# andrewendlinger/xmris

Measured on AMD Instinct MI355X. Metric: spectra/sec (zero_fill->apodize->FFT->autophase), n_time=4096; HBM-roofline %, higher is better.
Workload: dtype f32

## Files before the change

xmris_amd/csrc/xm_coarse.h:

```cpp
#pragma once
#include "xm_kernels.h"

typedef _Float16 xm_h8 __attribute__((ext_vector_type(8)));
typedef _Float16 xm_h2 __attribute__((ext_vector_type(2)));
typedef float xm_f16v __attribute__((ext_vector_type(16)));

struct CoarseArgs {
  const void* in;
  const float* window;
  const Cx<float>* w1024;
  float* est;
  unsigned long long* gkey;
  long long in_stride;
  long long n_batch;
  float scale2;
};

constexpr int kCoarseWaves = 4;

XM_DEV Cx<float> coarse_w1024(const Cx<float>* __restrict__ t, unsigned k) {
  k &= 1023u;
  const Cx<float> w = t[k & 511u];
  return (k & 512u) ? mk<float>(-w.re, -w.im) : w;
}

XM_DEV xm_h8 coarse_pack(const float* v) {
  union {
    xm_h8 v8;
    xm_h2 v2[4];
  } u;
#pragma unroll
  for (int j = 0; j < 4; ++j) {
    const xm_f2 p = {v[2 * j], v[2 * j + 1]};
    u.v2[j] = __builtin_convertvector(p, xm_h2);
  }
  return u.v8;
}

template <bool IN64>
__global__ __launch_bounds__(64 * kCoarseWaves, 2) void k_coarse_mfma(CoarseArgs A) {
  const unsigned lane = threadIdx.x & 63u, r = lane & 31u, h = lane >> 5;
  const long long wave = (long long)blockIdx.x * kCoarseWaves + (threadIdx.x >> 6);
  const long long n_waves = (long long)gridDim.x * kCoarseWaves;

  xm_h8 b1r, b1i, b1n, a2r[2], a2i[2], a2n[2];
  {
    float cr[8], ci[8], cn[8];
#pragma unroll
    for (int j = 0; j < 8; ++j) {
      const Cx<float> w = coarse_w1024(A.w1024, 32u * ((8u * h + (unsigned)j) * r));
      cr[j] = w.re;
      ci[j] = w.im;
      cn[j] = -w.im;
    }
    b1r = coarse_pack(cr);
    b1i = coarse_pack(ci);
    b1n = coarse_pack(cn);
#pragma unroll
    for (int s = 0; s < 2; ++s) {
#pragma unroll
      for (int j = 0; j < 8; ++j) {
        const unsigned n2 = 16u * s + 8u * ((unsigned)j >> 2) + 4u * h + ((unsigned)j & 3u);
        const Cx<float> w = coarse_w1024(A.w1024, 32u * (n2 * r));
        cr[j] = w.re;
        ci[j] = w.im;
        cn[j] = -w.im;
      }
      a2r[s] = coarse_pack(cr);
      a2i[s] = coarse_pack(ci);
      a2n[s] = coarse_pack(cn);
    }
  }
  float twr[16], twi[16];
#pragma unroll
  for (int q = 0; q < 16; ++q) {
    const unsigned n2 = ((unsigned)q & 3u) + 8u * ((unsigned)q >> 2) + 4u * h;
    const Cx<float> w = coarse_w1024(A.w1024, n2 * r);
    twr[q] = w.re;
    twi[q] = w.im;
  }
  float wnd[8];
#pragma unroll
  for (int j = 0; j < 8; ++j) wnd[j] = A.window[32u * (8u * h + (unsigned)j) + r];

  auto fetch = [&](long long s, Cx<float>* x) {
    if constexpr (IN64) {
      const xm_d2* __restrict__ row = reinterpret_cast<const xm_d2*>(A.in) + s * A.in_stride;
#pragma unroll
      for (int j = 0; j < 8; ++j) {
        const xm_d2 v = __builtin_nontemporal_load(row + 32u * (8u * h + (unsigned)j) + r);
        x[j] = mk<float>((float)v.x, (float)v.y);
      }
      return;
    }
    const xm_f2* __restrict__ row = reinterpret_cast<const xm_f2*>(A.in) + s * A.in_stride;
#pragma unroll
    for (int j = 0; j < 8; ++j) {
      const xm_f2 v = __builtin_nontemporal_load(row + 32u * (8u * h + (unsigned)j) + r);
      x[j] = mk<float>(v.x, v.y);
    }
  };

  unsigned best_key = 0u, best_row = 0u;
  bool have = false;
  constexpr int DEPTH = 1;
  Cx<float> nx[DEPTH][8];
  long long s = wave;
#pragma unroll
  for (int d = 0; d < DEPTH; ++d)
    if (s + d * n_waves < A.n_batch) fetch(s + d * n_waves, nx[d]);
  auto one_row = [&](Cx<float>* cur, long long s) {
    float re[8], im[8];
    float m = 0.f;
#pragma unroll
    for (int j = 0; j < 8; ++j) {
      re[j] = cur[j].re * wnd[j];
      im[j] = cur[j].im * wnd[j];
      m = fmaxf(m, fmaxf(fabsf(re[j]), fabsf(im[j])));
    }
    if (s + DEPTH * n_waves < A.n_batch) fetch(s + DEPTH * n_waves, cur);
    unsigned e = (wave_reduce_u32<true>(__float_as_uint(m)) >> 23) & 0xffu;
    e = e > 253u ? 253u : (e < 1u ? 1u : e);
    const float up = __uint_as_float((254u - e) << 23);
    const float down = __uint_as_float(e << 23);
#pragma unroll
    for (int j = 0; j < 8; ++j) {
      re[j] *= up;
      im[j] *= up;
    }
    const xm_h8 ar = coarse_pack(re), ai = coarse_pack(im);
    xm_f16v d1r = {0.f}, d1i = {0.f};
    d1r = __builtin_amdgcn_mfma_f32_32x32x16_f16(ar, b1r, d1r, 0, 0, 0);
    d1r = __builtin_amdgcn_mfma_f32_32x32x16_f16(ai, b1n, d1r, 0, 0, 0);
    d1i = __builtin_amdgcn_mfma_f32_32x32x16_f16(ar, b1i, d1i, 0, 0, 0);
    d1i = __builtin_amdgcn_mfma_f32_32x32x16_f16(ai, b1r, d1i, 0, 0, 0);
    float zr[16], zi[16];
#pragma unroll
    for (int q = 0; q < 16; ++q) {
      zr[q] = d1r[q] * twr[q] - d1i[q] * twi[q];
      zi[q] = d1r[q] * twi[q] + d1i[q] * twr[q];
    }
    xm_f16v d2r = {0.f}, d2i = {0.f};
#pragma unroll
    for (int k = 0; k < 2; ++k) {
      const xm_h8 br = coarse_pack(zr + 8 * k), bi = coarse_pack(zi + 8 * k);
      d2r = __builtin_amdgcn_mfma_f32_32x32x16_f16(a2r[k], br, d2r, 0, 0, 0);
      d2r = __builtin_amdgcn_mfma_f32_32x32x16_f16(a2n[k], bi, d2r, 0, 0, 0);
      d2i = __builtin_amdgcn_mfma_f32_32x32x16_f16(a2r[k], bi, d2i, 0, 0, 0);
      d2i = __builtin_amdgcn_mfma_f32_32x32x16_f16(a2i[k], br, d2i, 0, 0, 0);
    }
    float bv = -1.f;
#pragma unroll
    for (int q = 0; q < 16; ++q) bv = fmaxf(bv, d2r[q] * d2r[q] + d2i[q] * d2i[q]);
    bv = amax_nan_if_unset(bv);
    bv = bv * (down * down) * A.scale2;
    const unsigned key = wave_reduce_u32<true>(bv != bv ? 0x7fc00000u : __float_as_uint(bv));
    const unsigned row = (unsigned)s;
    const bool take = !have || key > best_key;
    best_key = take ? key : best_key;
    best_row = take ? row : best_row;
    have = true;
    if (lane == 0u) A.est[s] = __uint_as_float(key);
  };
  for (; s < A.n_batch; s += DEPTH * n_waves) {
#pragma unroll
    for (int d = 0; d < DEPTH; ++d)
      if (s + d * n_waves < A.n_batch) one_row(nx[d], s + d * n_waves);
  }
  if (A.gkey && have && lane == 0u)
    atomicMax(A.gkey + (blockIdx.x % XM_KEY_SLOTS) * XM_KEY_STRIDE,
              ((unsigned long long)best_key << 32) | (unsigned long long)(0xffffffffu - best_row));
}
```

xmris_amd/device.py:

```python
from __future__ import annotations

import numpy as np

from . import _lib


def _torch():
    import torch

    return torch


def _dtype_code(x) -> int:
    torch = _torch()
    if x.dtype == torch.complex64:
        return _lib.XM_C64
    if x.dtype == torch.complex128:
        return _lib.XM_C128
    raise TypeError(f"xmris_amd kernels need complex64/complex128 data, got {x.dtype}")


def _real_dtype(x):
    torch = _torch()
    return torch.float32 if x.dtype == torch.complex64 else torch.float64


def _require_device(x):
    torch = _torch()
    if not isinstance(x, torch.Tensor):
        raise TypeError("expected a torch.Tensor resident on the GPU")
    if not x.is_cuda:
        raise RuntimeError(
            "xmris_amd has no CPU path: the tensor must live on a HIP device (use xmris_amd.to_device)"
        )


def _stream(x):
    torch = _torch()
    return torch.cuda.current_stream(x.device).cuda_stream


def to_device(a, device="cuda", dtype=None):
    torch = _torch()
    if isinstance(a, torch.Tensor):
        t = a
    else:
        a = np.asarray(a)
        if not np.iscomplexobj(a):
            a = a.astype(np.complex128 if a.dtype != np.float32 else np.complex64)
        t = torch.from_numpy(np.ascontiguousarray(a))
    if dtype is not None:
        t = t.to(dtype)
    if not t.is_complex():
        t = t.to(torch.complex128 if t.dtype == torch.float64 else torch.complex64)
    return t.to(device)


_HOST_STAGE = {}
_HOST_STAGE_BUFS = 4
_HOST_STAGE_LOCK = __import__("threading").Lock()


def to_host(x, chunk_bytes: int = 32 << 20):
    torch = _torch()
    x = x.detach()
    nbytes = x.numel() * x.element_size()
    if not x.is_cuda or nbytes < 4 * chunk_bytes:
        return x.cpu().numpy()
    with _HOST_STAGE_LOCK:
        return _to_host_staged(x.contiguous(), chunk_bytes)


def _to_host_staged(x, chunk_bytes: int):
    torch = _torch()
    from concurrent.futures import ThreadPoolExecutor

    nbytes = x.numel() * x.element_size()
    dev_idx = x.device.index or 0
    if dev_idx not in _HOST_STAGE:
        _HOST_STAGE[dev_idx] = ([torch.empty(chunk_bytes, dtype=torch.uint8, pin_memory=True)
                                 for _ in range(_HOST_STAGE_BUFS)],
                                torch.cuda.Stream(device=x.device), ThreadPoolExecutor(max_workers=_HOST_STAGE_BUFS))
    stage, side, pool = _HOST_STAGE[dev_idx]
    np_dtype = {torch.complex64: np.complex64, torch.complex128: np.complex128, torch.float32: np.float32,
                torch.float64: np.float64}.get(x.dtype)
    if np_dtype is None or chunk_bytes != stage[0].numel():
        return x.cpu().numpy()
    out = np.empty(tuple(x.shape), dtype=np_dtype)
    dst = out.reshape(-1).view(np.uint8)
    src = (torch.view_as_real(x) if x.is_complex() else x).reshape(-1).view(torch.uint8)
    stage_np = [b.numpy() for b in stage]
    side.wait_stream(torch.cuda.current_stream(x.device))
    pending = [None] * len(stage)

    def drain(ev, lo, n, k):
        ev.synchronize()
        np.copyto(dst[lo:lo + n], stage_np[k][:n])

    for i, lo in enumerate(range(0, nbytes, chunk_bytes)):
        k, n = i % len(stage), min(chunk_bytes, nbytes - lo)
        if pending[k] is not None:
            pending[k].result()
        with torch.cuda.stream(side):
            stage[k][:n].copy_(src[lo:lo + n], non_blocking=True)
            ev = torch.cuda.Event()
            ev.record(side)
        pending[k] = pool.submit(drain, ev, lo, n, k)
    for f in pending:
        if f is not None:
            f.result()
    x.record_stream(side)
    return out


def _rows(x, axis):
    nd = x.dim()
    axis = axis % nd
    xm = x.movedim(axis, -1) if axis != nd - 1 else x
    lead = tuple(xm.shape[:-1])
    n = xm.shape[-1]
    x2 = xm.reshape(-1, n)
    if not x2.is_contiguous():
        x2 = x2.contiguous()

    def restore(y2):
        y = y2.reshape(lead + (y2.shape[-1],))
        if axis != nd - 1:
            y = y.movedim(-1, axis).contiguous()
        return y

    return x2, restore


def _table(values, like, complex_table: bool):
    torch = _torch()
    if isinstance(values, torch.Tensor):
        t = values
    else:
        t = torch.from_numpy(np.ascontiguousarray(np.asarray(values)))
    want = like.dtype if complex_table else _real_dtype(like)
    return t.to(device=like.device, dtype=want).contiguous()


def zero_fill(x, axis: int, target_points: int, pad_left: int = 0):
    _require_device(x)
    torch = _torch()
    x2, restore = _rows(x, axis)
    nb, n_in = x2.shape
    out = torch.empty((nb, target_points), dtype=x.dtype, device=x.device)
    _lib.call("xm_zero_fill", x2.data_ptr(), out.data_ptr(), nb, n_in, target_points, pad_left,
              _dtype_code(x), _stream(x))
    return restore(out)


def apodize(x, axis: int, window):
    _require_device(x)
    torch = _torch()
    x2, restore = _rows(x, axis)
    nb, n = x2.shape
    w = _table(window, x, complex_table=False)
    if w.numel() != n:
        raise ValueError(f"window has {w.numel()} points, axis has {n}")
    out = torch.empty_like(x2)
    _lib.call("xm_apodize", x2.data_ptr(), out.data_ptr(), w.data_ptr(), nb, n, _dtype_code(x), _stream(x))
    return restore(out)


def zf_apod_supported(n_out: int, out_complex128: bool) -> bool:
    return int(n_out) * (8 if out_complex128 else 4) <= 96 * 1024


def zf_apod(x2, n_out: int, pad_left: int, window, promote: bool = False):
    _require_device(x2)
    torch = _torch()
    if x2.dim() != 2 or not x2.is_contiguous():
        raise ValueError("zf_apod expects a contiguous [n_batch, n_in] tensor")
    nb, n_in = x2.shape
    out_dt = torch.complex128 if (promote or x2.dtype == torch.complex128) else torch.complex64
    rd = torch.float64 if out_dt == torch.complex128 else torch.float32
    if isinstance(window, torch.Tensor):
        w = window.to(device=x2.device, dtype=rd).contiguous()
    else:
        w = torch.from_numpy(np.ascontiguousarray(np.asarray(window, dtype=np.float64))).to(device=x2.device, dtype=rd)
    if w.numel() != n_out:
        raise ValueError(f"window has {w.numel()} points, the zero-filled axis has {n_out}")
    out = torch.empty((nb, n_out), dtype=out_dt, device=x2.device)
    _lib.call("xm_zf_apod", x2.data_ptr(), n_in, out.data_ptr(), w.data_ptr(), nb, n_in, int(n_out), int(pad_left),
              _dtype_code(x2), _lib.XM_C128 if out_dt == torch.complex128 else _lib.XM_C64, _stream(x2))
    return out


def phase_apply(x, axis: int, table):
    _require_device(x)
    torch = _torch()
    x2, restore = _rows(x, axis)
    nb, n = x2.shape
    ph = _table(table, x, complex_table=True)
    if ph.numel() != n:
        raise ValueError(f"phase table has {ph.numel()} points, axis has {n}")
    out = torch.empty_like(x2)
    _lib.call("xm_phase_apply", x2.data_ptr(), out.data_ptr(), ph.data_ptr(), nb, n, _dtype_code(x),
              _stream(x))
    return restore(out)


def roll(x, axis: int, shift: int):
    _require_device(x)
    torch = _torch()
    x2, restore = _rows(x, axis)
    nb, n = x2.shape
    out = torch.empty_like(x2)
    _lib.call("xm_roll", x2.data_ptr(), out.data_ptr(), nb, n, int(shift) % n, _dtype_code(x), _stream(x))
    return restore(out)


def fft(x, axis: int, inverse: bool = False, ortho: bool = True, shift_in: bool = False,
        shift_out: bool = False):
    _require_device(x)
    torch = _torch()
    x2, restore = _rows(x, axis)
    nb, n = x2.shape
    if n == 1:
        return restore(x2.clone())
    flags = ((_lib.XM_FFT_INVERSE if inverse else 0) | (_lib.XM_FFT_ORTHO if ortho else 0)
             | (_lib.XM_FFT_SHIFT_IN if shift_in else 0) | (_lib.XM_FFT_SHIFT_OUT if shift_out else 0))
    out = torch.empty_like(x2)
    _lib.call("xm_fft1d_batched", x2.data_ptr(), out.data_ptr(), nb, n, flags, _dtype_code(x), _stream(x))
    return restore(out)


def slice_axis(x, axis: int, start: int):
    _require_device(x)
    idx = [slice(None)] * x.dim()
    idx[axis % x.dim()] = slice(int(start), None)
    return x[tuple(idx)].contiguous()


def shift_fractional(x, axis: int, start: int, table):
    _require_device(x)
    torch = _torch()
    x2, restore = _rows(x, axis)
    nb, n = x2.shape
    m = n - int(start)
    ph = _table(table, x, complex_table=True)
    if ph.numel() != m:
        raise ValueError(f"table has {ph.numel()} points, sliced axis has {m}")
    view = x2[:, int(start):]
    spec = torch.empty((nb, m), dtype=x.dtype, device=x.device)
    code, st = _dtype_code(x), _stream(x)
    _lib.call("xm_pipeline_fused", view.data_ptr(), n, spec.data_ptr(), None, ph.data_ptr(), nb, m, m, 0, 0,
              None, None, code, st)
    out = torch.empty_like(spec)
    _lib.call("xm_fft1d_batched", spec.data_ptr(), out.data_ptr(), nb, m, _lib.XM_FFT_INVERSE, code, st)
    return restore(out)


def baseline_als(x, axis: int, lam: float, p: float, n_iter: int):
    torch = _torch()
    if not isinstance(x, torch.Tensor) or not x.is_cuda:
        raise RuntimeError("xmris_amd has no CPU path: the tensor must live on a HIP device")
    is_complex = x.is_complex()
    if x.dtype in (torch.complex64, torch.float32):
        code = _lib.XM_C64
    elif x.dtype in (torch.complex128, torch.float64):
        code = _lib.XM_C128
    else:
        raise TypeError(f"baseline_als needs float32/float64 (complex) data, got {x.dtype}")
    x2, restore = _rows(x, axis)
    nb, n = x2.shape
    need = int(_lib.load().xm_baseline_als_workspace_bytes(nb, n))
    work = torch.empty(max(need // 8, 1), dtype=torch.float64, device=x.device)
    out = torch.empty((nb, n), dtype=torch.float64, device=x.device)
    _lib.call("xm_baseline_als", x2.data_ptr(), int(is_complex), nb, n, float(lam), float(p), int(n_iter),
              out.data_ptr(), work.data_ptr(), need, code, torch.cuda.current_stream(x.device).cuda_stream)
    return restore(out)


def amares_model(params, n: int, dt: float, t0: float):
    torch = _torch()
    _require_device(params)
    p = params.to(torch.float64).contiguous()
    if p.dim() < 2 or p.shape[-1] != 5:
        raise ValueError(f"amares_model needs parameters [..., n_peaks, 5], got {tuple(p.shape)}")
    lead, k = tuple(p.shape[:-2]), p.shape[-2]
    nb = int(np.prod(lead, dtype=np.int64)) if lead else 1
    out = torch.empty(lead + (n,), dtype=torch.complex128, device=p.device)
    _lib.call("xm_amares_model", p.data_ptr(), nb, k, int(n), float(dt), float(t0), out.data_ptr(), _stream(p))
    return out


class AmaresFit:

    __slots__ = ("params", "amp_sd", "rss", "status", "iters", "fit", "n_free")

    def __init__(self, **kw):
        for k, v in kw.items():
            setattr(self, k, v)


def amares_fit(x, axis: int, init, lo, hi, fixed, dt: float, t0: float = 0.0, max_iter: int = 200,
               ftol: float = 1e-10, xtol: float = 1e-10, want_fit: bool = True) -> AmaresFit:
    torch = _torch()
    _require_device(x)
    code = _dtype_code(x)
    init, lo, hi = (np.ascontiguousarray(np.asarray(v, dtype=np.float64).reshape(-1, 5)) for v in (init, lo, hi))
    fixed = np.ascontiguousarray(np.asarray(fixed, dtype=bool).reshape(-1, 5).astype(np.int32))
    k = init.shape[0]
    if not (lo.shape == hi.shape == fixed.shape == init.shape):
        raise ValueError("init, lo, hi and fixed must all be [n_peaks, 5]")
    axis = axis % x.dim()
    x2, restore = _rows(x, axis)
    nb, n = x2.shape
    lead = tuple(s for i, s in enumerate(x.shape) if i != axis)
    dev_ = x.device
    params = torch.empty((nb, k, 5), dtype=torch.float64, device=dev_)
    asd = torch.empty((nb, k), dtype=torch.float64, device=dev_)
    rss = torch.empty(nb, dtype=torch.float64, device=dev_)
    status = torch.empty(nb, dtype=torch.int32, device=dev_)
    iters = torch.empty(nb, dtype=torch.int32, device=dev_)
    fit = torch.empty((nb, n), dtype=torch.complex128, device=dev_) if want_fit else None
    need = int(_lib.load().xm_amares_workspace_bytes(nb, n, k))
    work = torch.zeros(max(need, 8), dtype=torch.uint8, device=dev_)
    ptr = lambda a: a.ctypes.data
    _lib.call("xm_amares_fit", x2.data_ptr(), n, nb, n, float(dt), float(t0), k, ptr(init), ptr(lo), ptr(hi), ptr(fixed),
              int(max_iter), float(ftol), float(xtol), params.data_ptr(), asd.data_ptr(), rss.data_ptr(),
              status.data_ptr(), iters.data_ptr(), fit.data_ptr() if fit is not None else None, work.data_ptr(), need,
              code, _stream(x))
    n_free = int(np.count_nonzero(~(fixed.astype(bool) | (lo == hi))))
    return AmaresFit(params=params.reshape(lead + (k, 5)), amp_sd=asd.reshape(lead + (k,)), rss=rss.reshape(lead),
                     status=status.reshape(lead), iters=iters.reshape(lead),
                     fit=fit.reshape(lead + (n,)) if fit is not None else None, n_free=n_free)


def absmax_argmax(x):
    _require_device(x)
    torch = _torch()
    xc = x if x.is_contiguous() else x.contiguous()
    n = xc.shape[-1] if xc.dim() else 1
    x2 = xc.reshape(-1, n)
    nb = x2.shape[0]
    rd = _real_dtype(x)
    amax = torch.empty(nb, dtype=rd, device=x.device)
    aidx = torch.empty(nb, dtype=torch.int32, device=x.device)
    gmax = torch.empty(1, dtype=rd, device=x.device)
    gflat = torch.empty(1, dtype=torch.int64, device=x.device)
    code, st = _dtype_code(x), _stream(x)
    _lib.call("xm_absmax_rows", x2.data_ptr(), nb, n, amax.data_ptr(), aidx.data_ptr(), code, st)
    _lib.call("xm_argmax_reduce", amax.data_ptr(), aidx.data_ptr(), nb, n, gmax.data_ptr(), gflat.data_ptr(),
              code, st)
    return float(gmax.item()) ** 0.5, int(gflat.item())


class FusedResult:

    __slots__ = ("out", "absmax2", "argidx")

    def __init__(self, out, absmax2, argidx):
        self.out, self.absmax2, self.argidx = out, absmax2, argidx


def ramp_native(x2, n_out: int, pad_left: int = 0, shift_out: bool = True, ortho: bool = True) -> bool:
    _require_device(x2)
    flags = (_lib.XM_FFT_ORTHO if ortho else 0) | (_lib.XM_FFT_SHIFT_OUT if shift_out else 0)
    return bool(_lib.load().xm_pipeline_ramp_native(x2.data_ptr(), x2.shape[1], x2.shape[1], int(n_out), int(pad_left),
                                                    flags, _dtype_code(x2)))


def key_native(x2, n_out: int, pad_left: int = 0, shift_out: bool = True, ortho: bool = True) -> bool:
    _require_device(x2)
    flags = (_lib.XM_FFT_ORTHO if ortho else 0) | (_lib.XM_FFT_SHIFT_OUT if shift_out else 0)
    return x2.shape[0] >= 2 and bool(_lib.load().xm_pipeline_key_native(x2.data_ptr(), x2.shape[1], x2.shape[1], int(n_out),
                                                                       int(pad_left), flags, _dtype_code(x2)))


def pipeline_fused(x2, n_out: int, pad_left: int = 0, window=None, phase_table=None, shift_out: bool = True,
                   ortho: bool = True, want_out: bool = True, want_argmax: bool = False, out=None,
                   absmax2=None, argidx=None, argmax_value_only: bool = False, phase_ramp=None, global_key=None,
                   key_result=None):
    _require_device(x2)
    torch = _torch()
    if x2.dim() != 2 or not x2.is_contiguous():
        raise ValueError("pipeline_fused expects a contiguous [n_batch, n_in] tensor")
    nb, n_in = x2.shape
    rd = _real_dtype(x2)
    if want_out and out is None:
        out = torch.empty((nb, n_out), dtype=x2.dtype, device=x2.device)
    if global_key is not None:
        want_argmax, absmax2 = True, global_key
        argidx = key_result
    if want_argmax:
        if absmax2 is None:
            absmax2 = torch.empty(nb, dtype=rd, device=x2.device)
        if argidx is None and global_key is None:
            argidx = torch.empty(nb, dtype=torch.int32, device=x2.device)
    flags = (_lib.XM_FFT_ORTHO if ortho else 0) | (_lib.XM_FFT_SHIFT_OUT if shift_out else 0)
    if global_key is not None:
        flags |= _lib.XM_AMAX_GLOBAL_KEY | _lib.XM_AMAX_VALUE_ONLY
    if argmax_value_only:
        flags |= _lib.XM_AMAX_VALUE_ONLY
    if phase_ramp is not None:
        if phase_table is not None or not want_out:
            raise ValueError("phase_ramp excludes phase_table and needs an output")
        _lib.call(
            "xm_pipeline_fused_ramp", x2.data_ptr(), n_in, out.data_ptr(),
            window.data_ptr() if window is not None else None, float(phase_ramp[0]), float(phase_ramp[1]), nb, n_in,
            n_out, pad_left, flags, absmax2.data_ptr() if want_argmax else None,
            argidx.data_ptr() if (want_argmax and argidx is not None) else None, _dtype_code(x2), _stream(x2))
        return FusedResult(out, absmax2 if want_argmax else None, argidx if want_argmax else None)
    _lib.call(
        "xm_pipeline_fused", x2.data_ptr(), n_in, out.data_ptr() if want_out else None,
        window.data_ptr() if window is not None else None,
        phase_table.data_ptr() if phase_table is not None else None, nb, n_in, n_out, pad_left, flags,
        absmax2.data_ptr() if want_argmax else None,
        argidx.data_ptr() if (want_argmax and argidx is not None) else None, _dtype_code(x2), _stream(x2))
    return FusedResult(out if want_out else None, absmax2 if want_argmax else None,
                       argidx if want_argmax else None)


def row_l1(x2, window=None, pad_left: int = 0, out=None, n_used: int | None = None, sub_step: int = 1, key=None):
    _require_device(x2)
    torch = _torch()
    if x2.dim() != 2 or not x2.is_contiguous():
        raise ValueError("row_l1 expects a contiguous [n_batch, n_in] tensor")
    nb, n_in = x2.shape
    if out is None and key is None:
        out = torch.empty(nb, dtype=_real_dtype(x2), device=x2.device)
    n_sum = n_in if n_used is None else max(1, min(int(n_used), n_in))
    _lib.call("xm_row_l1", x2.data_ptr(), n_in, window.data_ptr() if window is not None else None, nb, n_sum,
              int(pad_left), max(1, int(sub_step)), out.data_ptr() if out is not None else None,
              key.data_ptr() if key is not None else None, _dtype_code(x2), _stream(x2))
    return out


def guess_supported(x2, n_out: int, pad_left: int = 0, shift_out: bool = True, ortho: bool = True) -> bool:
    _require_device(x2)
    if x2.dim() != 2 or not x2.is_contiguous():
        return False
    flags = (_lib.XM_FFT_ORTHO if ortho else 0) | (_lib.XM_FFT_SHIFT_OUT if shift_out else 0)
    return bool(_lib.load().xm_guess_supported(x2.data_ptr(), x2.shape[1], x2.shape[1], int(n_out), int(pad_left), flags,
                                               _dtype_code(x2)))


def guess_rows(x2, n_out: int, window32, est, key, n_guess: int = 0, shift_out: bool = True, ortho: bool = True):
    _require_device(x2)
    flags = (_lib.XM_FFT_ORTHO if ortho else 0) | (_lib.XM_FFT_SHIFT_OUT if shift_out else 0)
    nb, n_in = x2.shape
    _lib.call("xm_guess_rows", x2.data_ptr(), n_in, window32.data_ptr() if window32 is not None else None, nb, n_in,
              int(n_out), int(n_guess), flags, est.data_ptr(), key.data_ptr(), _dtype_code(x2), _stream(x2))
    return est


def guess_refine(x2, n_out: int, window32, est, guess_key, work_key, gmax, gflat, out_row, band: float = 0.75,
                 shift_out: bool = True, ortho: bool = True):
    _require_device(x2)
    flags = (_lib.XM_FFT_ORTHO if ortho else 0) | (_lib.XM_FFT_SHIFT_OUT if shift_out else 0)
    nb, n_in = x2.shape
    _lib.call("xm_guess_refine", x2.data_ptr(), n_in, window32.data_ptr() if window32 is not None else None, nb, n_in,
              int(n_out), flags, est.data_ptr(), guess_key.data_ptr(), float(band), work_key.data_ptr(),
              gmax.data_ptr(), gflat.data_ptr(), out_row.data_ptr(), _dtype_code(x2), _stream(x2))
    return out_row


def new_argmax_key(device):
    return _torch().zeros(131072 // 8, dtype=_torch().int64, device=device)


def new_key_result():
    return _torch().zeros(2, dtype=_torch().int64, pin_memory=True)


def read_key_result(rec, complex128: bool = False):
    m2 = rec.view(_torch().float64)[0] if complex128 else rec.view(_torch().float32)[0]
    return float(m2.item()), int(rec[1].item())


def argmax_key_take(key, n_per_row: int, gmax, gflat, x2=None, out_row=None):
    torch = _torch()
    if x2 is not None:
        _require_device(x2)
        if out_row is None:
            out_row = torch.empty((1, x2.shape[1]), dtype=torch.complex128, device=x2.device)
    st = torch.cuda.current_stream(key.device).cuda_stream
    _lib.call("xm_argmax_key_take", key.data_ptr(), int(n_per_row), gmax.data_ptr(), gflat.data_ptr(),
              x2.data_ptr() if x2 is not None else None, x2.shape[1] if x2 is not None else 0,
              x2.shape[1] if x2 is not None else 0, out_row.data_ptr() if x2 is not None else None,
              _dtype_code(x2) if x2 is not None else _lib.XM_C64, st)
    return out_row


def argmax_reduce(absmax2, argidx, n: int):
    torch = _torch()
    nb = absmax2.numel()
    gmax = torch.empty(1, dtype=absmax2.dtype, device=absmax2.device)
    gflat = torch.empty(1, dtype=torch.int64, device=absmax2.device)
    code = _lib.XM_C64 if absmax2.dtype == torch.float32 else _lib.XM_C128
    _lib.call("xm_argmax_reduce", absmax2.data_ptr(), argidx.data_ptr(), nb, n, gmax.data_ptr(),
              gflat.data_ptr(), code, torch.cuda.current_stream(absmax2.device).cuda_stream)
    return float(gmax.item()) ** 0.5, int(gflat.item())


def argmax_reduce_async(absmax2, argidx, n: int, gmax=None, gflat=None):
    torch = _torch()
    nb = absmax2.numel()
    if gmax is None:
        gmax = torch.empty(1, dtype=absmax2.dtype, device=absmax2.device)
    if gflat is None:
        gflat = torch.empty(1, dtype=torch.int64, device=absmax2.device)
    code = _lib.XM_C64 if absmax2.dtype == torch.float32 else _lib.XM_C128
    _lib.call("xm_argmax_reduce", absmax2.data_ptr(), argidx.data_ptr(), nb, n, gmax.data_ptr(),
              gflat.data_ptr(), code, torch.cuda.current_stream(absmax2.device).cuda_stream)
    return gmax, gflat


def gather_row_c128(x2, gflat, n_per_row: int, out=None):
    _require_device(x2)
    torch = _torch()
    nb, n_in = x2.shape
    if out is None:
        out = torch.empty((1, n_in), dtype=torch.complex128, device=x2.device)
    _lib.call("xm_gather_row_c128", x2.data_ptr(), n_in, n_in, gflat.data_ptr(), int(n_per_row), out.data_ptr(),
              _dtype_code(x2), _stream(x2))
    return out


def last_kernel() -> str:
    v = _lib.load().xm_last_kernel_string()
    return v.decode("utf-8", "replace") if v else ""


def fft_supported(n: int, complex128: bool = False) -> bool:
    if n == 1:
        return True
    return bool(_lib.load().xm_fft_supported(int(n), _lib.XM_C128 if complex128 else _lib.XM_C64))


SEARCH_RECORD_WORDS = 16


def search_supported(n: int, method: str = "acme", x_range: float = 1.0) -> bool:
    from .autophase_solver import METHODS

    return method in METHODS and bool(_lib.load().xm_search_supported(int(n), METHODS.index(method), float(x_range)))


def new_search_record():
    return _torch().zeros(SEARCH_RECORD_WORDS, dtype=_torch().int64, pin_memory=True)


def uniform_axis(coords):
    c = np.asarray(coords, dtype=np.float64)
    if c.size < 2:
        return None
    step = (c[-1] - c[0]) / (c.size - 1)
    rng = float(c.max() - c.min())
    if step == 0 or rng <= 0 or not np.all(np.abs(c - (c[0] + step * np.arange(c.size))) <= 4e-15 * rng):
        return None
    return float(c[0]), float(step), rng


def search_launch(slice_c128, axis, record, seq: int, p0_only: bool = False, seed: int = 42, tol: float = 0.01,
                  maxiter: int = 1000, stream=None):
    torch = _torch()
    n = slice_c128.numel()
    st = (stream if stream is not None else torch.cuda.current_stream()).cuda_stream
    _lib.call("xm_search_launch", slice_c128.data_ptr(), int(n), float(axis[0]), float(axis[1]), float(axis[2]), 0,
              int(bool(p0_only)), int(seed), float(tol), int(maxiter), int(seq), record.data_ptr(), st)


def search_done(record, seq: int) -> bool:
    return int(_lib.load().xm_atomic_load_acquire_i64(record.data_ptr() + 56)) == int(seq)


def read_search_record(record) -> dict:
    f = record.view(_torch().float64)
    i = record.view(_torch().int32)
    return dict(x=(float(f[0]), float(f[1])), fun=float(f[2]), pg_norm=float(f[3]), nfev=int(i[8]), nit=int(i[9]),
                status=int(i[10]), needs_polish=bool(int(i[11])), target_idx=int(i[12]),
                t_us=[float(v) for v in f[8:14]])


def search_eval(slice_c128, axis, xs, target_idx: int = -1, p0_only: bool = False):
    torch = _torch()
    xs_t = torch.as_tensor(np.ascontiguousarray(xs, dtype=np.float64)).reshape(-1, 2).to(slice_c128.device if slice_c128.is_cuda else "cuda")
    fs = torch.empty(xs_t.shape[0], dtype=torch.float64, device=xs_t.device)
    _lib.call("xm_search_eval", slice_c128.data_ptr(), int(slice_c128.numel()), float(axis[0]), float(axis[1]),
              float(axis[2]), int(target_idx), int(bool(p0_only)), xs_t.data_ptr(), int(xs_t.shape[0]), fs.data_ptr(),
              torch.cuda.current_stream().cuda_stream)
    return fs.cpu().numpy()


class ChipPartition:

    def __init__(self, device, reserved: int, n_search: int):
        import ctypes

        torch = _torch()
        self.device, self.reserved = device, int(reserved)
        self._handles = []

        def make(partition):
            h = ctypes.c_void_p()
            with torch.cuda.device(device):
                _lib.call("xm_stream_create", ctypes.byref(h), int(reserved), partition)
            self._handles.append(h.value)
            return torch.cuda.ExternalStream(h.value, device=device)

        self.compute = make(0)
        self.search = [make(1) for _ in range(int(n_search))]

    def another_search_stream(self):
        import ctypes

        h = ctypes.c_void_p()
        with _torch().cuda.device(self.device):
            _lib.call("xm_stream_create", ctypes.byref(h), self.reserved, 1)
        self._handles.append(h.value)
        st = _torch().cuda.ExternalStream(h.value, device=self.device)
        self.search.append(st)
        return st


_PARTITIONS = {}


def chip_partition(device, reserved: int, n_search: int) -> ChipPartition:
    torch = _torch()
    device = torch.device(device)
    key = (device.index if device.index is not None else torch.cuda.current_device(), int(reserved))
    part = _PARTITIONS.get(key)
    if part is None:
        part = _PARTITIONS[key] = ChipPartition(device, reserved, n_search)
    while len(part.search) < n_search:
        part.another_search_stream()
    return part


def replacement_search_stream(device, partition_streams):
    torch = _torch()
    if partition_streams is None:
        return torch.cuda.Stream(device=device)
    for part in _PARTITIONS.values():
        if partition_streams and partition_streams[0] in part.search:
            return part.another_search_stream()
    return torch.cuda.Stream(device=device)
```

Measured before the change: 57.90 million.

## Stage coarse-pass rows through LDS with 16-byte loads and track per-block top candidates

The complex64 coarse kernel now reads each row with wide 16-byte loads into a per-wave LDS strip, then reads it back in the strided layout the MFMA operands need, replacing eight 8-byte strided loads per lane. It also keeps a per-wave top-16 candidate list in registers via ballot/shuffle, merges it per block in shared memory, and writes the records plus a header into an enlarged key buffer. Tuning macros for occupancy, prefetch depth and nontemporal loads are added. The candidate bookkeeping adds per-row shuffle work, extra LDS, and a larger key buffer.

```diff
diff --git a/xmris_amd/csrc/xm_cand.h b/xmris_amd/csrc/xm_cand.h
--- /dev/null
+++ b/xmris_amd/csrc/xm_cand.h
@@ -0,0 +1,72 @@
+#pragma once
+#include <stddef.h>
+#include <stdint.h>
+
+typedef unsigned long long xm_ckey;
+
+#if defined(__HIPCC__)
+#define XM_HD __host__ __device__ inline
+#else
+#define XM_HD inline
+#endif
+
+constexpr int XM_CAND_CAP = 16;
+constexpr int XM_KEY_LIST_WORD = 6144;
+constexpr int XM_KEY_LIST_BYTE = 131072;
+constexpr int XM_KEY_LIST_MAX = 1024;
+constexpr uint32_t XM_KEY_LIST_TAG = 0x4c495354u;
+constexpr uint32_t XM_CAND_NAN = 0x7fc00000u;
+
+XM_HD xm_ckey xm_cand_key(uint32_t est_bits, uint32_t row) {
+  const uint32_t e = (est_bits & 0x7fffffffu) > 0x7f800000u ? XM_CAND_NAN : est_bits;
+  return ((xm_ckey)e << 32) | (xm_ckey)(0xffffffffu - row);
+}
+XM_HD uint32_t xm_cand_row(xm_ckey k) { return 0xffffffffu - (uint32_t)(k & 0xffffffffu); }
+XM_HD uint32_t xm_cand_est_bits(xm_ckey k) { return (uint32_t)(k >> 32); }
+
+XM_HD float xm_cand_bits_to_float(uint32_t b) {
+  union {
+    uint32_t u;
+    float f;
+  } c;
+  c.u = b;
+  return c.f;
+}
+
+XM_HD bool xm_cand_in_band(xm_ckey k, float thr) {
+  const float e = xm_cand_bits_to_float(xm_cand_est_bits(k));
+  return k != 0u && (e >= thr || e != e);
+}
+
+XM_HD void xm_cand_insert(xm_ckey* list, xm_ckey k) {
+  if (k <= list[XM_CAND_CAP - 1]) return;
+  int pos = XM_CAND_CAP - 1;
+  while (pos > 0 && list[pos - 1] < k) {
+    list[pos] = list[pos - 1];
+    --pos;
+  }
+  list[pos] = k;
+}
+
+XM_HD unsigned xm_cand_rank(const xm_ckey* all, unsigned n, unsigned i) {
+  const xm_ckey mine = all[i];
+  unsigned r = 0;
+  for (unsigned j = 0; j < n; ++j) r += (all[j] > mine || (all[j] == mine && j < i)) ? 1u : 0u;
+  return r;
+}
+
+XM_HD unsigned xm_cand_merge(const xm_ckey* records, unsigned n_rec, float thr, xm_ckey* out) {
+  for (int i = 0; i < XM_CAND_CAP; ++i) out[i] = 0u;
+  for (unsigned r = 0; r < n_rec; ++r)
+    for (int i = 0; i < XM_CAND_CAP; ++i) {
+      const xm_ckey k = records[(size_t)r * XM_CAND_CAP + i];
+      if (xm_cand_in_band(k, thr)) xm_cand_insert(out, k);
+    }
+  unsigned n = 0;
+  while (n < (unsigned)XM_CAND_CAP && out[n] != 0u) ++n;
+  return n;
+}
+
+XM_HD unsigned xm_cand_block_of_row(xm_ckey row, unsigned n_blocks, unsigned waves_per_block) {
+  return (unsigned)(row % ((xm_ckey)n_blocks * waves_per_block)) / waves_per_block;
+}
diff --git a/xmris_amd/csrc/xm_coarse.h b/xmris_amd/csrc/xm_coarse.h
--- a/xmris_amd/csrc/xm_coarse.h
+++ b/xmris_amd/csrc/xm_coarse.h
@@ -1,4 +1,5 @@
 #pragma once
+#include "xm_cand.h"
 #include "xm_kernels.h"
 
 typedef _Float16 xm_h8 __attribute__((ext_vector_type(8)));
@@ -17,6 +18,18 @@
 };
 
 constexpr int kCoarseWaves = 4;
+#ifndef XM_COARSE_WGS
+#define XM_COARSE_WGS 2
+#endif
+#ifndef XM_COARSE_DEPTH
+#define XM_COARSE_DEPTH 1
+#endif
+#ifndef XM_COARSE_L16
+#define XM_COARSE_L16 1
+#endif
+#ifndef XM_COARSE_NT
+#define XM_COARSE_NT 1
+#endif
 
 XM_DEV Cx<float> coarse_w1024(const Cx<float>* __restrict__ t, unsigned k) {
   k &= 1023u;
@@ -38,8 +51,11 @@
 }
 
 template <bool IN64>
-__global__ __launch_bounds__(64 * kCoarseWaves, 2) void k_coarse_mfma(CoarseArgs A) {
+__global__ __launch_bounds__(64 * kCoarseWaves, XM_COARSE_WGS) void k_coarse_mfma(CoarseArgs A) {
   const unsigned lane = threadIdx.x & 63u, r = lane & 31u, h = lane >> 5;
+  constexpr bool L16 = !IN64 && XM_COARSE_L16;
+  __shared__ __attribute__((aligned(16))) unsigned long long strip[kCoarseWaves][L16 ? 512 : XM_CAND_CAP];
+  unsigned long long* my_strip = strip[threadIdx.x >> 6];
   const long long wave = (long long)blockIdx.x * kCoarseWaves + (threadIdx.x >> 6);
   const long long n_waves = (long long)gridDim.x * kCoarseWaves;
 
@@ -83,39 +99,71 @@
 #pragma unroll
   for (int j = 0; j < 8; ++j) wnd[j] = A.window[32u * (8u * h + (unsigned)j) + r];
 
-  auto fetch = [&](long long s, Cx<float>* x) {
+  struct Raw {
+    xm_u4 q[4];
+    Cx<float> x[L16 ? 1 : 8];
+  };
+  auto fetch = [&](long long s, Raw& w) {
     if constexpr (IN64) {
       const xm_d2* __restrict__ row = reinterpret_cast<const xm_d2*>(A.in) + s * A.in_stride;
 #pragma unroll
       for (int j = 0; j < 8; ++j) {
         const xm_d2 v = __builtin_nontemporal_load(row + 32u * (8u * h + (unsigned)j) + r);
-        x[j] = mk<float>((float)v.x, (float)v.y);
-      }
-      return;
-    }
-    const xm_f2* __restrict__ row = reinterpret_cast<const xm_f2*>(A.in) + s * A.in_stride;
-#pragma unroll
-    for (int j = 0; j < 8; ++j) {
-      const xm_f2 v = __builtin_nontemporal_load(row + 32u * (8u * h + (unsigned)j) + r);
-      x[j] = mk<float>(v.x, v.y);
+        w.x[j] = mk<float>((float)v.x, (float)v.y);
+      }
+    } else if constexpr (L16) {
+      const xm_u4* __restrict__ row = reinterpret_cast<const xm_u4*>(reinterpret_cast<const xm_f2*>(A.in) + s * A.in_stride);
+#pragma unroll
+      for (int i = 0; i < 4; ++i) w.q[i] = XM_COARSE_NT ? __builtin_nontemporal_load(row + 64u * i + lane) : row[64u * i + lane];
+    } else {
+      const xm_f2* __restrict__ row = reinterpret_cast<const xm_f2*>(A.in) + s * A.in_stride;
+#pragma unroll
+      for (int j = 0; j < 8; ++j) {
+        const xm_f2 v = XM_COARSE_NT ? __builtin_nontemporal_load(row + 32u * (8u * h + (unsigned)j) + r) : row[32u * (8u * h + (unsigned)j) + r];
+        w.x[j] = mk<float>(v.x, v.y);
+      }
+    }
+  };
+  auto operand = [&](const Raw& w, Cx<float>* x) {
+    if constexpr (L16) {
+      xm_u4* wr = reinterpret_cast<xm_u4*>(my_strip);
+#pragma unroll
+      for (int i = 0; i < 4; ++i) wr[64u * i + lane] = w.q[i];
+      __builtin_amdgcn_fence(__ATOMIC_RELEASE, "wavefront");
+      __builtin_amdgcn_wave_barrier();
+      __builtin_amdgcn_fence(__ATOMIC_ACQUIRE, "wavefront");
+      const xm_f2* rd = reinterpret_cast<const xm_f2*>(my_strip);
+#pragma unroll
+      for (int j = 0; j < 8; ++j) {
+        const xm_f2 v = rd[32u * (8u * h + (unsigned)j) + r];
+        x[j] = mk<float>(v.x, v.y);
+      }
+      __builtin_amdgcn_fence(__ATOMIC_RELEASE, "wavefront");
+      __builtin_amdgcn_wave_barrier();
+    } else {
+#pragma unroll
+      for (int j = 0; j < 8; ++j) x[j] = w.x[j];
     }
   };
 
   unsigned best_key = 0u, best_row = 0u;
   bool have = false;
-  constexpr int DEPTH = 1;
-  Cx<float> nx[DEPTH][8];
+  unsigned long long top = 0ull, top_min = 0ull;
+  constexpr int DEPTH = XM_COARSE_DEPTH;
+  Raw nx[DEPTH];
   long long s = wave;
 #pragma unroll
   for (int d = 0; d < DEPTH; ++d)
     if (s + d * n_waves < A.n_batch) fetch(s + d * n_waves, nx[d]);
-  auto one_row = [&](Cx<float>* cur, long long s) {
+  auto one_row = [&](Raw& cur, long long s) {
     float re[8], im[8];
     float m = 0.f;
+    Cx<float> x[8];
+    operand(cur, x);
 #pragma unroll
     for (int j = 0; j < 8; ++j) {
-      re[j] = cur[j].re * wnd[j];
-      im[j] = cur[j].im * wnd[j];
+      re[j] = x[j].re * wnd[j];
+      im[j] = x[j].im * wnd[j];
       m = fmaxf(m, fmaxf(fabsf(re[j]), fabsf(im[j])));
     }
     if (s + DEPTH * n_waves < A.n_batch) fetch(s + DEPTH * n_waves, cur);
@@ -161,6 +209,13 @@
     best_row = take ? row : best_row;
     have = true;
     if (lane == 0u) A.est[s] = __uint_as_float(key);
+    const unsigned long long ck = xm_cand_key(key, row);
+    if (ck > top_min) {
+      const unsigned pos = (unsigned)__builtin_popcountll(__ballot(lane < (unsigned)XM_CAND_CAP && top > ck));
+      const unsigned long long up = __shfl_up(top, 1, XM_WAVE);
+      top = lane < pos ? top : (lane == pos ? ck : up);
+      top_min = __shfl(top, XM_CAND_CAP - 1, XM_WAVE);
+    }
   };
   for (; s < A.n_batch; s += DEPTH * n_waves) {
 #pragma unroll
@@ -170,4 +225,23 @@
   if (A.gkey && have && lane == 0u)
     atomicMax(A.gkey + (blockIdx.x % XM_KEY_SLOTS) * XM_KEY_STRIDE,
               ((unsigned long long)best_key << 32) | (unsigned long long)(0xffffffffu - best_row));
+  if (A.gkey) {
+    __syncthreads();
+    unsigned long long* all = strip[0];
+    if (lane < (unsigned)XM_CAND_CAP) all[(threadIdx.x >> 6) * XM_CAND_CAP + lane] = top;
+    __syncthreads();
+    if (threadIdx.x < (unsigned)(kCoarseWaves * XM_CAND_CAP)) {
+      const unsigned rank = xm_cand_rank(all, kCoarseWaves * XM_CAND_CAP, threadIdx.x);
+      unsigned long long* rec = reinterpret_cast<unsigned long long*>(reinterpret_cast<char*>(A.gkey) + XM_KEY_LIST_BYTE) +
+                                (size_t)blockIdx.x * XM_CAND_CAP;
+      if (rank < (unsigned)XM_CAND_CAP) rec[rank] = all[threadIdx.x];
+    }
+    if (blockIdx.x == 0u && threadIdx.x == 0u) {
+      unsigned* hdr = reinterpret_cast<unsigned*>(A.gkey) + XM_KEY_LIST_WORD;
+      hdr[0] = XM_KEY_LIST_TAG;
+      hdr[1] = gridDim.x;
+      hdr[2] = (unsigned)(unsigned long long)A.n_batch;
+      hdr[3] = (unsigned)((unsigned long long)A.n_batch >> 32);
+    }
+  }
 }
diff --git a/xmris_amd/device.py b/xmris_amd/device.py
--- a/xmris_amd/device.py
+++ b/xmris_amd/device.py
@@ -462,7 +462,7 @@
 
 
 def new_argmax_key(device):
-    return _torch().zeros(131072 // 8, dtype=_torch().int64, device=device)
+    return _torch().zeros(262144 // 8, dtype=_torch().int64, device=device)
 
 
 def new_key_result():
```

Measured after the change: 57.92 million (median of 5 runs). No clear change (+0.0%).
